# gsgen3d/gsgen

Hardware: AMD Instinct MI355X
Metric: fwd+bwd renders/sec (800x800, 100k Gaussians) (higher is better)
Workload: dtype f32

## Files before the change

### gsgen_amd/csrc/binning.hip

```cpp
#include "common.hpp"
#include "../../include/gsgen_hip.h"
#include <cstdlib>
#include <vector>

#if defined(GSGEN_EMU_KNOBS)
extern "C" unsigned long long gsgen_emu_emit_staged_keys;
unsigned long long gsgen_emu_emit_staged_keys = 0;
#endif

namespace gs {

constexpr int kGroup = 8;
constexpr int kChunk = 2048;

struct GroupGeom {
  int gx0, gy0, tx, ty, tile;
  bool in_grid;
};
__device__ __forceinline__ GroupGeom group_geom(int ntw, int nth) {
  const int ngw = (ntw + kGroup - 1) / kGroup;
  const int g = (int)blockIdx.x;
  GroupGeom q;
  q.gx0 = (g % ngw) * kGroup;
  q.gy0 = (g / ngw) * kGroup;
  const int lane = lane_id();
  q.tx = q.gx0 + (lane & 7);
  q.ty = q.gy0 + (lane >> 3);
  q.in_grid = (q.tx < ntw) && (q.ty < nth);
  q.tile = q.ty * ntw + q.tx;
  return q;
}

constexpr int kPullWaves = 4;
constexpr int kIter = kChunk / (64 * kPullWaves);

__device__ __forceinline__ int rd_lane(int v, int l) { return __builtin_amdgcn_readlane(v, l); }

struct RectRegs {
  int x0[kIter], y0[kIter], x1[kIter], y1[kIter];
};

template <bool EMIT>
__device__ __forceinline__ void
bin_pull_body(uint32_t N, const int *__restrict__ tl, const int *__restrict__ br,
           const float *__restrict__ depth, int ntw, int nth, uint32_t T,
           uint32_t *__restrict__ cnt, uint32_t *__restrict__ wcnt, const uint32_t *__restrict__ tile_off,
           const uint32_t *__restrict__ ctrl, unsigned long long *__restrict__ keys) {
  __shared__ uint32_t s_cnt[kPullWaves][64];
  if (EMIT && ctrl[1] != 0u) return;
  const GroupGeom q = group_geom(ntw, nth);
  const uint32_t chunk = blockIdx.y;
  const int lane = lane_id();
  const int wave = (int)(threadIdx.x >> 6);
  const uint32_t begin = chunk * (uint32_t)kChunk + (uint32_t)wave * (uint32_t)(64 * kIter);
  const uint32_t stop = min(N, chunk * (uint32_t)kChunk + (uint32_t)kChunk);

  RectRegs R;
  unsigned dbits[EMIT ? kIter : 1];
  unsigned long long touch[kIter];
#pragma unroll
  for (int it = 0; it < kIter; ++it) {
    const uint32_t i = begin + (uint32_t)(it * 64 + lane);
    int x0 = 0, y0 = 0, x1 = -1, y1 = -1;
    if (i < stop) {
      const int2 a = *reinterpret_cast<const int2 *>(tl + 2 * (size_t)i);
      const int2 c = *reinterpret_cast<const int2 *>(br + 2 * (size_t)i);
      x0 = max(a.x, 0); y0 = max(a.y, 0); x1 = min(c.x, ntw - 1); y1 = min(c.y, nth - 1);
      if (EMIT) dbits[it] = __float_as_uint(depth[i]);
    } else if (EMIT) {
      dbits[it] = 0u;
    }
    const bool touches = (x1 >= x0) && (y1 >= y0) && (x1 >= q.gx0) && (x0 <= q.gx0 + kGroup - 1) &&
                         (y1 >= q.gy0) && (y0 <= q.gy0 + kGroup - 1);
    touch[it] = __ballot(touches);
    R.x0[it] = x0; R.y0[it] = y0; R.x1[it] = x1; R.y1[it] = y1;
  }
  if (!EMIT) {
    uint32_t running = 0;
#pragma unroll
    for (int it = 0; it < kIter; ++it) {
      unsigned long long m = touch[it];
      while (m != 0ull) {
        const int src = __ffsll((long long)m) - 1;
        m &= (m - 1ull);
        const int rx0 = rd_lane(R.x0[it], src), rx1 = rd_lane(R.x1[it], src);
        const int ry0 = rd_lane(R.y0[it], src), ry1 = rd_lane(R.y1[it], src);
        const bool hit = (q.tx >= rx0) && (q.tx <= rx1) && (q.ty >= ry0) && (q.ty <= ry1);
        running += hit ? 1u : 0u;
      }
    }
    if (q.in_grid) wcnt[((size_t)chunk * kPullWaves + (size_t)wave) * T + q.tile] = running;
    s_cnt[wave][lane] = running;
    __syncthreads();
    if (wave == 0 && q.in_grid)
      cnt[(size_t)chunk * T + q.tile] = s_cnt[0][lane] + s_cnt[1][lane] + s_cnt[2][lane] + s_cnt[3][lane];
    return;
  }
  uint32_t pos = 0;
  if (q.in_grid) {
    pos = tile_off[q.tile] + cnt[(size_t)chunk * T + q.tile];
    for (int w = 0; w < wave; ++w) pos += wcnt[((size_t)chunk * kPullWaves + (size_t)w) * T + q.tile];
  }
#pragma unroll
  for (int it = 0; it < kIter; ++it) {
    unsigned long long m = touch[it];
    const uint32_t i0 = begin + (uint32_t)(it * 64);
    while (m != 0ull) {
      const int src = __ffsll((long long)m) - 1;
      m &= (m - 1ull);
      const int rx0 = rd_lane(R.x0[it], src), rx1 = rd_lane(R.x1[it], src);
      const int ry0 = rd_lane(R.y0[it], src), ry1 = rd_lane(R.y1[it], src);
      const bool hit = (q.tx >= rx0) && (q.tx <= rx1) && (q.ty >= ry0) && (q.ty <= ry1);
      const unsigned db = (unsigned)rd_lane((int)dbits[EMIT ? it : 0], src);
      if (hit) {
        keys[pos] = ((unsigned long long)db << 32) | (unsigned long long)(i0 + (uint32_t)src);
        ++pos;
      }
    }
  }
}

constexpr uint32_t kScanChunkTiles = 64;
template <uint32_t NW>
__device__ __forceinline__ void
scan_chunks_body(uint32_t T, uint32_t nchunks, uint32_t *__restrict__ cnt, uint32_t *__restrict__ tile_count) {
  __shared__ uint32_t s_part[NW][kScanChunkTiles];
  const uint32_t lane = (uint32_t)lane_id(), w = threadIdx.x >> 6;
  const uint32_t t = blockIdx.x * kScanChunkTiles + lane;
  const uint32_t q = (nchunks + NW - 1u) / NW;
  const uint32_t c0 = min(w * q, nchunks), c1 = min(c0 + q, nchunks);
  uint32_t sum = 0;
  if (t < T)
    for (uint32_t c = c0; c < c1; ++c) sum += cnt[(size_t)c * T + t];
  s_part[w][lane] = sum;
  __syncthreads();
  uint32_t run = 0;
  for (uint32_t k = 0; k < w; ++k) run += s_part[k][lane];
  if (t < T) {
    for (uint32_t c = c0; c < c1; ++c) {
      const uint32_t v = cnt[(size_t)c * T + t];
      cnt[(size_t)c * T + t] = run;
      run += v;
    }
    if (w == NW - 1u) tile_count[t] = run;
  }
}

__device__ __forceinline__ uint32_t sat_add_u32(uint32_t a, uint32_t b) {
  const uint32_t s = a + b;
  return s < a ? 0xffffffffu : s;
}

constexpr uint32_t kScanThreads = 256;
__device__ __forceinline__ void report_pair_count(uint32_t *report, uint32_t total, bool overflow) {
  if (report == nullptr) return;
#if defined(__HIP_DEVICE_COMPILE__)
  __hip_atomic_store(report, total, __ATOMIC_RELAXED, __HIP_MEMORY_SCOPE_SYSTEM);
  if (overflow) __hip_atomic_fetch_max(report + 1, total, __ATOMIC_RELAXED, __HIP_MEMORY_SCOPE_SYSTEM);
#else
  report[0] = total;
  if (overflow && report[1] < total) report[1] = total;
#endif
}
__device__ __forceinline__ void
scan_tiles_body(uint32_t T, const uint32_t *__restrict__ tile_count, uint32_t *__restrict__ tile_off,
             uint32_t *__restrict__ ctrl, uint32_t cap, uint32_t *__restrict__ total_out, uint32_t *report = nullptr) {
  __shared__ uint32_t s_part[kScanThreads];
  const uint32_t t = threadIdx.x;
  const uint32_t per = (T + kScanThreads - 1u) / kScanThreads;
  const uint32_t b = min(t * per, T), e = min(b + per, T);
  uint32_t sum = 0;
  for (uint32_t i = b; i < e; ++i) sum = sat_add_u32(sum, tile_count[i]);
  s_part[t] = sum;
  __syncthreads();
  for (uint32_t d = 1; d < kScanThreads; d <<= 1) {
    const uint32_t v = (t >= d) ? s_part[t - d] : 0u;
    __syncthreads();
    s_part[t] = sat_add_u32(s_part[t], v);
    __syncthreads();
  }
  uint32_t run = (t > 0) ? s_part[t - 1] : 0u;
  for (uint32_t i = b; i < e; ++i) {
    tile_off[i] = run;
    run = sat_add_u32(run, tile_count[i]);
  }
  if (t == kScanThreads - 1u) {
    const uint32_t total = s_part[kScanThreads - 1u];
    tile_off[T] = total;
    ctrl[0] = total;
    ctrl[1] = (total > cap) ? 1u : 0u;
    if (total_out != nullptr) *total_out = total;
    report_pair_count(report, total, total > cap);
  }
}

constexpr uint32_t kWaveSortMax = 512;
__device__ __forceinline__ void
order_tiles_body(uint32_t T, const uint32_t *__restrict__ tile_count, uint32_t *__restrict__ tile_order, uint32_t *__restrict__ n_long) {
  __shared__ uint32_t s_hist[256];
  __shared__ uint32_t s_base[256];
  const uint32_t t = threadIdx.x;
  if (t < 256u) s_hist[t] = 0u;
  __syncthreads();
  for (uint32_t i = t; i < T; i += kScanThreads) atomicAdd(&s_hist[255u - min(tile_count[i] >> 3, 255u)], 1u);
  __syncthreads();
  if (t == 0) {
    uint32_t run = 0;
    for (int b = 0; b < 256; ++b) {
      if (b == 256 - (int)(kWaveSortMax >> 3)) *n_long = run;
      s_base[b] = run;
      run += s_hist[b];
    }
  }
  __syncthreads();
  for (uint32_t i = t; i < T; i += kScanThreads) {
    const uint32_t b = 255u - min(tile_count[i] >> 3, 255u);
    tile_order[atomicAdd(&s_base[b], 1u)] = i;
  }
}

typedef unsigned long long u64;
__device__ __forceinline__ void cmpx(u64 &lo, u64 &hi) {
  const u64 a = lo, b = hi;
  const bool sw = a > b;
  lo = sw ? b : a;
  hi = sw ? a : b;
}
template <int K>
__device__ __forceinline__ void cross_step(u64 (&k)[K], int m, bool flip) {
  const int lane = lane_id();
  int top = m;
  top |= top >> 1; top |= top >> 2; top |= top >> 4;
  top = (top + 1) >> 1;
  const bool upper = (lane & top) != 0;
  auto pick = [&](u64 mine, u64 theirs) {
    const bool take = (theirs < mine) != upper;
    const uint32_t lo = take ? (uint32_t)theirs : (uint32_t)mine, hi = take ? (uint32_t)(theirs >> 32) : (uint32_t)(mine >> 32);
    return ((u64)hi << 32) | lo;
  };
  if (flip) {
    if constexpr (K == 1) {
      k[0] = pick(k[0], __shfl_xor(k[0], m, 64));
    } else {
#pragma unroll
      for (int r = 0; r < K / 2; ++r) {
        const u64 a = k[r], b = k[K - 1 - r];
        const u64 oa = __shfl_xor(b, m, 64), ob = __shfl_xor(a, m, 64);
        k[r] = pick(a, oa);
        k[K - 1 - r] = pick(b, ob);
      }
    }
  } else {
#pragma unroll
    for (int r = 0; r < K; ++r) k[r] = pick(k[r], __shfl_xor(k[r], m, 64));
  }
}
template <int K, int J>
__device__ __forceinline__ void local_step(u64 (&k)[K]) {
#pragma unroll
  for (int r = 0; r < K; ++r) {
    if ((r & J) == 0) cmpx(k[r], k[r | J]);
  }
}
template <int K, int J>
__device__ __forceinline__ void local_tail(u64 (&k)[K]) {
  if constexpr (J >= 1) {
    local_step<K, J>(k);
    local_tail<K, J / 2>(k);
  }
}
template <int K, int SIZE>
__device__ __forceinline__ void local_sizes(u64 (&k)[K]) {
  if constexpr (SIZE <= K) {
#pragma unroll
    for (int r = 0; r < K; ++r) {
      const int l = r ^ (SIZE - 1);
      if (l > r) cmpx(k[r], k[l]);
    }
    local_tail<K, SIZE / 4>(k);
    local_sizes<K, SIZE * 2>(k);
  }
}
template <int K>
__device__ __forceinline__ void sort_regs(u64 (&k)[K]) {
  local_sizes<K, 2>(k);
  for (int size = 2 * K; size <= 64 * K; size <<= 1) {
    cross_step<K>(k, size / K - 1, true);
    for (int j = size >> 2; j >= K; j >>= 1) cross_step<K>(k, j / K, false);
    local_tail<K, K / 2>(k);
  }
}
template <int K>
__device__ __forceinline__ void sort_segment_regs(const u64 *__restrict__ keys, int *__restrict__ ids, uint32_t n) {
  const uint32_t lane = (uint32_t)lane_id();
  u64 k[K];
#pragma unroll
  for (int r = 0; r < K; ++r) {
    const uint32_t e = lane * K + r;
    k[r] = (e < n) ? keys[e] : ~0ull;
  }
  sort_regs<K>(k);
#pragma unroll
  for (int r = 0; r < K; ++r) {
    const uint32_t e = lane * K + r;
    if (e < n) ids[e] = (int)(uint32_t)(k[r] & 0xffffffffull);
  }
}
__device__ __forceinline__ void long_pass(u64 *__restrict__ k, uint32_t n, uint32_t p2, uint32_t dist, bool flip) {
  const uint32_t lane = (uint32_t)lane_id();
  const uint32_t half = p2 >> 1;
  for (uint32_t cbase = 0; cbase < half; cbase += 256u) {
    u64 a[4], b[4];
    uint32_t ia[4], ib[4];
#pragma unroll
    for (int u = 0; u < 4; ++u) {
      const uint32_t c = cbase + (uint32_t)u * 64u + lane;
      const uint32_t off = c & (dist - 1u);
      ia[u] = ((c - off) << 1) + off;
      ib[u] = flip ? (ia[u] ^ (2u * dist - 1u)) : (ia[u] + dist);
      const bool live = c < half && ib[u] < n;
      if (!live) ib[u] = 0xffffffffu;
      a[u] = live ? k[ia[u]] : 0ull;
      b[u] = live ? k[ib[u]] : ~0ull;
    }
#pragma unroll
    for (int u = 0; u < 4; ++u)
      if (ib[u] != 0xffffffffu && a[u] > b[u]) { k[ia[u]] = b[u]; k[ib[u]] = a[u]; }
  }
  wave_mem_fence();
}
template <int K>
__device__ __forceinline__ void sort_segment_long(u64 *__restrict__ keys, int *__restrict__ ids, uint32_t n) {
  constexpr uint32_t kBlock = 64u * K;
  const uint32_t lane = (uint32_t)lane_id();
  const uint32_t nblk = (n + kBlock - 1u) / kBlock;
  u64 k[K];
  for (uint32_t blk = 0; blk < nblk; ++blk) {
    const uint32_t e0 = blk * kBlock + lane * K;
#pragma unroll
    for (int r = 0; r < K; ++r) k[r] = (e0 + r < n) ? keys[e0 + r] : ~0ull;
    sort_regs<K>(k);
    if (nblk == 1u) {
#pragma unroll
      for (int r = 0; r < K; ++r)
        if (e0 + r < n) ids[e0 + r] = (int)(uint32_t)(k[r] & 0xffffffffull);
      return;
    }
#pragma unroll
    for (int r = 0; r < K; ++r)
      if (e0 + r < n) keys[e0 + r] = k[r];
  }
  wave_mem_fence();
  uint32_t p2 = kBlock;
  while (p2 < n) p2 <<= 1;
  for (uint32_t size = 2u * kBlock; size <= p2; size <<= 1) {
    long_pass(keys, n, p2, size >> 1, true);
    for (uint32_t j = size >> 2; j >= kBlock; j >>= 1) long_pass(keys, n, p2, j, false);
    const bool last = size == p2;
    for (uint32_t blk = 0; blk < nblk; ++blk) {
      const uint32_t e0 = blk * kBlock + lane * K;
#pragma unroll
      for (int r = 0; r < K; ++r) k[r] = (e0 + r < n) ? keys[e0 + r] : ~0ull;
      for (int j = (int)kBlock / 2; j >= K; j >>= 1) cross_step<K>(k, j / K, false);
      local_tail<K, K / 2>(k);
#pragma unroll
      for (int r = 0; r < K; ++r) {
        if (e0 + r < n) {
          if (last) ids[e0 + r] = (int)(uint32_t)(k[r] & 0xffffffffull);
          else keys[e0 + r] = k[r];
        }
      }
    }
    wave_mem_fence();
  }
}

constexpr int kCoopWaves = 4;
constexpr uint32_t kCoopMax = 2048;
__device__ __forceinline__ void lds_pass(u64 *k, uint32_t p2, uint32_t dist, bool flip) {
  for (uint32_t c = threadIdx.x; c < (p2 >> 1); c += 64u * kCoopWaves) {
    const uint32_t off = c & (dist - 1u);
    const uint32_t i = ((c - off) << 1) + off;
    const uint32_t l = flip ? (i ^ (2u * dist - 1u)) : (i + dist);
    const u64 a = k[i], b = k[l];
    if (a > b) { k[i] = b; k[l] = a; }
  }
  __syncthreads();
}
template <int KW>
__device__ __forceinline__ void sort_segment_coop(const u64 *__restrict__ keys, int *__restrict__ ids, uint32_t n, u64 *s_keys) {
  constexpr uint32_t kBlk = 64u * KW;
  const uint32_t wave = threadIdx.x >> 6, lane = (uint32_t)lane_id();
  const uint32_t e0 = wave * kBlk + lane * KW;
  u64 k[KW];
#pragma unroll
  for (int r = 0; r < KW; ++r) k[r] = (e0 + r < n) ? keys[e0 + r] : ~0ull;
  sort_regs<KW>(k);
  auto to_lds = [&]() {
#pragma unroll
    for (int r = 0; r < KW; ++r) s_keys[e0 + r] = k[r];
    __syncthreads();
  };
  auto tail_in_registers = [&]() {
#pragma unroll
    for (int r = 0; r < KW; ++r) k[r] = s_keys[e0 + r];
    for (int j = (int)kBlk / 2; j >= KW; j >>= 1) cross_step<KW>(k, j / KW, false);
    local_tail<KW, KW / 2>(k);
  };
  to_lds();
  lds_pass(s_keys, 4u * kBlk, kBlk, true);
  tail_in_registers();
  __syncthreads();
  to_lds();
  lds_pass(s_keys, 4u * kBlk, 2u * kBlk, true);
  lds_pass(s_keys, 4u * kBlk, kBlk, false);
  tail_in_registers();
#pragma unroll
  for (int r = 0; r < KW; ++r)
    if (e0 + r < n) ids[e0 + r] = (int)(uint32_t)(k[r] & 0xffffffffull);
}
__device__ __forceinline__ void
sort_tiles_coop_body(uint32_t tile, const uint32_t *__restrict__ tile_off, const uint32_t *__restrict__ ctrl,
                     unsigned long long *__restrict__ keys, int *__restrict__ ids, int *__restrict__ start,
                     int *__restrict__ end, u64 *s_keys) {
  const uint32_t tid = threadIdx.x;
  if (ctrl[1] != 0u) {
    if (tid == 0) { start[tile] = kListOverflow; end[tile] = kListOverflow; }
    return;
  }
  const uint32_t b = tile_off[tile], e = tile_off[tile + 1];
  const uint32_t n = e - b;
  if (tid == 0) {
    start[tile] = n ? (int)b : -1;
    end[tile] = n ? (int)e : -1;
  }
  if (n == 0) return;
  if (n <= 256u || n > kCoopMax) {
    if (tid >= 64u) return;
    if (n <= 64u) sort_segment_regs<1>(keys + b, ids + b, n);
    else if (n <= 128u) sort_segment_regs<2>(keys + b, ids + b, n);
    else if (n <= 256u) sort_segment_regs<4>(keys + b, ids + b, n);
    else sort_segment_long<8>(keys + b, ids + b, n);
    return;
  }
  if (n <= 512u) sort_segment_coop<2>(keys + b, ids + b, n, s_keys);
  else if (n <= 1024u) sort_segment_coop<4>(keys + b, ids + b, n, s_keys);
  else sort_segment_coop<8>(keys + b, ids + b, n, s_keys);
}
__device__ __forceinline__ void
sort_tiles_packed_body(uint32_t slot, uint32_t T, const uint32_t *__restrict__ tile_order, const uint32_t *__restrict__ tile_off,
                       const uint32_t *__restrict__ ctrl, unsigned long long *__restrict__ keys, int *__restrict__ ids,
                       int *__restrict__ start, int *__restrict__ end, u64 *s_keys) {
  const uint32_t n_long = min(ctrl[2], T);
  if (slot < n_long) {
    sort_tiles_coop_body(tile_order[slot], tile_off, ctrl, keys, ids, start, end, s_keys);
    return;
  }
  const uint32_t at = n_long + (slot - n_long) * (uint32_t)kCoopWaves + (threadIdx.x >> 6);
  if (at >= T) return;
  const uint32_t tile = tile_order[at];
  const bool first = lane_id() == 0;
  if (ctrl[1] != 0u) {
    if (first) { start[tile] = kListOverflow; end[tile] = kListOverflow; }
    return;
  }
  const uint32_t b = tile_off[tile], e = tile_off[tile + 1];
  const uint32_t n = e - b;
  if (first) {
    start[tile] = n ? (int)b : -1;
    end[tile] = n ? (int)e : -1;
  }
  if (n == 0) return;
  if (n <= 64u) sort_segment_regs<1>(keys + b, ids + b, n);
  else if (n <= 128u) sort_segment_regs<2>(keys + b, ids + b, n);
  else if (n <= 256u) sort_segment_regs<4>(keys + b, ids + b, n);
  else sort_segment_regs<8>(keys + b, ids + b, n);
}
static_assert(kWaveSortMax <= 512 && kWaveSortMax % 8 == 0 && kWaveSortMax <= 255 * 8, "sort_tiles_packed_body");
__global__ void __launch_bounds__(64 * kCoopWaves)
k_sort_tiles(uint32_t T, const uint32_t *__restrict__ tile_off, const uint32_t *__restrict__ ctrl,
                  unsigned long long *__restrict__ keys, int *__restrict__ ids, int *__restrict__ start,
                  int *__restrict__ end, const uint32_t *__restrict__ tile_order) {
  __shared__ u64 s_keys[kCoopMax];
  if (tile_order != nullptr) sort_tiles_packed_body(blockIdx.x, T, tile_order, tile_off, ctrl, keys, ids, start, end, s_keys);
  else sort_tiles_coop_body(blockIdx.x, tile_off, ctrl, keys, ids, start, end, s_keys);
}
__global__ void __launch_bounds__(64 * kCoopWaves)
k_sort_tiles_views(uint32_t T, uint32_t B, const GeoView *__restrict__ views) {
  __shared__ u64 s_keys[kCoopMax];
  const uint32_t rank = blockIdx.x / B;
  const GeoView v = views[blockIdx.x - rank * B];
  sort_tiles_packed_body(rank, T, v.tile_order, v.tile_off, v.ctrl, v.keys, v.ids, v.start, v.end, s_keys);
}

template <bool EMIT>
__global__ void __launch_bounds__(64 * kPullWaves)
k_bin_pull(uint32_t N, const int *__restrict__ tl, const int *__restrict__ br,
           const float *__restrict__ depth, int ntw, int nth, uint32_t T,
           uint32_t *__restrict__ cnt, uint32_t *__restrict__ wcnt, const uint32_t *__restrict__ tile_off,
           const uint32_t *__restrict__ ctrl, unsigned long long *__restrict__ keys) {
  bin_pull_body<EMIT>(N, tl, br, depth, ntw, nth, T, cnt, wcnt, tile_off, ctrl, keys);
}
template <bool EMIT>
__global__ void __launch_bounds__(64 * kPullWaves)
k_bin_pull_views(uint32_t N, int ntw, int nth, uint32_t T, const GeoView *__restrict__ views) {
  const GeoView v = views[blockIdx.z];
  bin_pull_body<EMIT>(N, v.tl, v.br, v.depth, ntw, nth, T, v.cnt, v.wcnt, v.tile_off, v.ctrl, v.keys);
}
__global__ void __launch_bounds__(1024)
k_scan_chunks(uint32_t T, uint32_t nchunks, uint32_t *__restrict__ cnt, uint32_t *__restrict__ tile_count) {
  scan_chunks_body<16>(T, nchunks, cnt, tile_count);
}
__global__ void __launch_bounds__(256)
k_scan_chunks_views(uint32_t T, uint32_t nchunks, const GeoView *__restrict__ views) {
  const GeoView v = views[blockIdx.y];
  scan_chunks_body<4>(T, nchunks, v.cnt, v.tile_count);
}
__global__ void __launch_bounds__(kScanThreads)
k_scan_order_tiles(uint32_t T, const uint32_t *__restrict__ tile_count, uint32_t *__restrict__ tile_off,
                   uint32_t *__restrict__ ctrl, uint32_t cap, uint32_t *__restrict__ total_out,
                   uint32_t *__restrict__ tile_order, uint32_t *report) {
  scan_tiles_body(T, tile_count, tile_off, ctrl, cap, total_out, report);
  order_tiles_body(T, tile_count, tile_order, ctrl + 2);
}
__global__ void __launch_bounds__(kScanThreads)
k_scan_order_tiles_views(uint32_t T, const GeoView *__restrict__ views) {
  const GeoView v = views[blockIdx.y];
  scan_tiles_body(T, v.tile_count, v.tile_off, v.ctrl, v.cap, v.total, v.report);
  order_tiles_body(T, v.tile_count, v.tile_order, v.ctrl + 2);
}
constexpr int kPushOwn = 12;
constexpr uint32_t kPushMaxTiles = 8192;
constexpr int kPushThreads = 512;
constexpr uint32_t kPushMinWorkgroups = 128;
constexpr uint32_t kPushMinWorkgroupsBatch = 32;
static uint32_t push_min_workgroups(bool batch) {
#if defined(GSGEN_EMU_KNOBS)
  if (const char *e = getenv("GSGEN_BIN_PUSH_MIN_WORKGROUPS")) return (uint32_t)strtoul(e, nullptr, 10);
#endif
  return batch ? kPushMinWorkgroupsBatch : kPushMinWorkgroups;
}
#if !defined(GSGEN_EMIT_STAGE_WORDS)
#define GSGEN_EMIT_STAGE_WORDS 12288
#endif
constexpr uint32_t kEmitStageWords = GSGEN_EMIT_STAGE_WORDS;
constexpr int kEmitIdBits = 11;
static_assert(kChunk == (1 << kEmitIdBits) && kPushMaxTiles <= (1u << (32 - kEmitIdBits)), "a staged word is (tile << 11) | local id");
static_assert(kPushMaxTiles % kPushThreads == 0 && kPushThreads % 64 == 0, "bin_push_body");
#if defined(__HIP_DEVICE_COMPILE__)
#define GS_PUSH_COUNTERS(name) extern __shared__ uint32_t name[]
#else
#define GS_PUSH_COUNTERS(name) __shared__ uint32_t name[kPushMaxTiles + kEmitAuxWords + kEmitStageWords]
#endif
constexpr uint32_t kEmitLdsWords = 16384;
constexpr uint32_t kEmitAuxWords = 16;
static_assert(kPushThreads / 64 <= 14 && kPushMaxTiles + kEmitAuxWords + 64 <= kEmitLdsWords && kEmitStageWords >= 64, "bin_push_body");
__host__ __device__ __forceinline__ uint32_t emit_stage_cap(uint32_t T) { return min(kEmitStageWords, kEmitLdsWords - kEmitAuxWords - T); }
static size_t push_lds_bytes(uint32_t T, bool emit) { return sizeof(uint32_t) * ((size_t)T + (emit ? kEmitAuxWords + emit_stage_cap(T) : 0u)); }
template <bool EMIT>
__device__ __forceinline__ void
bin_push_body(uint32_t N, const int *__restrict__ tl, const int *__restrict__ br, const float *__restrict__ depth, int ntw, int nth,
              uint32_t T, uint32_t *__restrict__ cnt, const uint32_t *__restrict__ tile_count, const uint32_t *__restrict__ tile_off,
              const uint32_t *__restrict__ ctrl, unsigned long long *__restrict__ keys, uint32_t *s_tile) {
  if (EMIT && ctrl[1] != 0u) return;
  const uint32_t chunk = blockIdx.x;
  const uint32_t chunk_base = chunk * (uint32_t)kChunk;
  uint32_t *const crow = cnt + (size_t)chunk * T;
  uint32_t *const s_wsum = s_tile + T, *const s_meta = s_wsum + 14, *const s_stage = s_wsum + kEmitAuxWords;
  const uint32_t stage_cap = emit_stage_cap(T);
  const int lane = lane_id();
  uint32_t n_staged_tiles = 0, n_staged = 0;
  if constexpr (EMIT) {
    const uint32_t *const nrow = (chunk + 1u < gridDim.x) ? crow + T : tile_count;
    for (uint32_t t = threadIdx.x; t < T; t += (uint32_t)kPushThreads) s_tile[t] = nrow[t] - crow[t];
    if (threadIdx.x < 2u) s_meta[threadIdx.x] = 0u;
    __syncthreads();
    const uint32_t per = (T + (uint32_t)kPushThreads - 1u) / (uint32_t)kPushThreads;
    const uint32_t b = min(threadIdx.x * per, T), e = min(b + per, T);
    uint32_t sum = 0;
    for (uint32_t i = b; i < e; ++i) sum += s_tile[i];
    uint32_t inc = sum;
    for (int d = 1; d < 64; d <<= 1) {
      const uint32_t v = __shfl(inc, max(lane - d, 0), 64);
      if (lane >= d) inc += v;
    }
    const uint32_t wave = threadIdx.x >> 6;
    if (lane == 63) s_wsum[wave] = inc;
    __syncthreads();
    uint32_t run = inc - sum;
    for (uint32_t w = 0; w < wave; ++w) run += s_wsum[w];
    uint32_t last_tile = 0, last_end = 0;
    for (uint32_t i = b; i < e; ++i) {
      const uint32_t c = s_tile[i];
      if (run + c <= stage_cap) {
        s_tile[i] = run;
        last_tile = i + 1u; last_end = run + c;
      } else {
        s_tile[i] = tile_off[i] + crow[i];
      }
      run += c;
    }
    if (last_tile != 0u) { atomicMax(&s_meta[0], last_tile); atomicMax(&s_meta[1], last_end); }
    __syncthreads();
    n_staged_tiles = s_meta[0]; n_staged = s_meta[1];
  } else {
    for (uint32_t t = threadIdx.x; t < T; t += (uint32_t)kPushThreads) s_tile[t] = 0u;
    __syncthreads();
  }
  const uint32_t stop = min(N, chunk_base + (uint32_t)kChunk);
  auto visit = [&](int tile, uint32_t id, unsigned dbits) {
    const uint32_t pos = atomicAdd(&s_tile[tile], 1u);
    if (EMIT) {
      if ((uint32_t)tile < n_staged_tiles) {
        if (pos < stage_cap) s_stage[pos] = ((uint32_t)tile << kEmitIdBits) | (id - chunk_base);
      } else {
        keys[pos] = ((unsigned long long)dbits << 32) | (unsigned long long)id;
      }
    }
  };
  for (uint32_t i0 = chunk_base; i0 < stop; i0 += (uint32_t)kPushThreads) {
    const uint32_t i = i0 + threadIdx.x;
    int x0 = 0, y0 = 0, x1 = -1, y1 = -1;
    unsigned db = 0u;
    if (i < stop) {
      const int2 a = *reinterpret_cast<const int2 *>(tl + 2 * (size_t)i);
      const int2 c = *reinterpret_cast<const int2 *>(br + 2 * (size_t)i);
      x0 = max(a.x, 0); y0 = max(a.y, 0); x1 = min(c.x, ntw - 1); y1 = min(c.y, nth - 1);
      if (EMIT) db = __float_as_uint(depth[i]);
    }
    const int rw = x1 - x0 + 1, rh = y1 - y0 + 1;
    const int n = (rw > 0 && rh > 0) ? rw * rh : 0;
    {
      int tx = x0, ty = y0;
      const int own = min(n, kPushOwn);
      for (int k = 0; k < own; ++k) {
        visit(ty * ntw + tx, i, db);
        if (++tx > x1) { tx = x0; ++ty; }
      }
    }
    unsigned long long big = __ballot(n > kPushOwn);
    while (big != 0ull) {
      const int src = __ffsll((long long)big) - 1;
      big &= (big - 1ull);
      const int bx0 = rd_lane(x0, src), by0 = rd_lane(y0, src), bw = rd_lane(rw, src), bn = rd_lane(n, src);
      const uint32_t bid = (uint32_t)rd_lane((int)i, src);
      const unsigned bdb = (unsigned)rd_lane((int)db, src);
      for (int k = kPushOwn + lane; k < bn; k += 64) {
        const int ry = k / bw;
        visit((by0 + ry) * ntw + bx0 + (k - ry * bw), bid, bdb);
      }
    }
  }
  __syncthreads();
  if constexpr (!EMIT) {
    for (uint32_t t = threadIdx.x; t < T; t += (uint32_t)kPushThreads) crow[t] = s_tile[t];
  } else {
    constexpr int kPer = (int)kPushMaxTiles / kPushThreads;
    uint32_t prev[kPer];
#pragma unroll
    for (int k = 0; k < kPer; ++k) {
      const uint32_t t = threadIdx.x + (uint32_t)(k * kPushThreads);
      prev[k] = (t > 0u && t < n_staged_tiles) ? s_tile[t - 1u] : 0u;
    }
    __syncthreads();
#pragma unroll
    for (int k = 0; k < kPer; ++k) {
      const uint32_t t = threadIdx.x + (uint32_t)(k * kPushThreads);
      if (t < n_staged_tiles) s_tile[t] = tile_off[t] + crow[t] - prev[k];
    }
    __syncthreads();
#if defined(GSGEN_EMU_KNOBS)
    if (threadIdx.x == 0) gsgen_emu_emit_staged_keys += n_staged;
#endif
    for (uint32_t j = threadIdx.x; j < n_staged; j += (uint32_t)kPushThreads) {
      const uint32_t w = s_stage[j];
      const uint32_t id = chunk_base + (w & ((1u << kEmitIdBits) - 1u));
      keys[j + s_tile[w >> kEmitIdBits]] = ((unsigned long long)__float_as_uint(depth[id]) << 32) | (unsigned long long)id;
    }
  }
}

template <bool EMIT>
__global__ void __launch_bounds__(kPushThreads)
k_bin_push(uint32_t N, const int *__restrict__ tl, const int *__restrict__ br, const float *__restrict__ depth, int ntw, int nth,
           uint32_t T, uint32_t *__restrict__ cnt, const uint32_t *__restrict__ tile_count, const uint32_t *__restrict__ tile_off,
           const uint32_t *__restrict__ ctrl, unsigned long long *__restrict__ keys) {
  GS_PUSH_COUNTERS(s_tile);
  bin_push_body<EMIT>(N, tl, br, depth, ntw, nth, T, cnt, tile_count, tile_off, ctrl, keys, s_tile);
}
template <bool EMIT>
__global__ void __launch_bounds__(kPushThreads)
k_bin_push_views(uint32_t N, int ntw, int nth, uint32_t T, const GeoView *__restrict__ views) {
  GS_PUSH_COUNTERS(s_tile);
  const GeoView v = views[blockIdx.y];
  bin_push_body<EMIT>(N, v.tl, v.br, v.depth, ntw, nth, T, v.cnt, v.tile_count, v.tile_off, v.ctrl, v.keys, s_tile);
}

template <int P>
__global__ void __launch_bounds__(64) k_selftest_reduce_scatter(const float *__restrict__ in, float *__restrict__ out) {
  float v[P];
  const int lane = lane_id();
#pragma unroll
  for (int i = 0; i < P; ++i) v[i] = in[lane * P + i];
  wave_reduce_scatter<P>(v);
  out[lane] = v[0];
  out[64 + lane] = (float)(scatter_owner<P>(lane) ? scatter_comp<P>(lane) : -1);
}

__global__ void __launch_bounds__(64) k_selftest_reduce_scatter_sep16(const float *__restrict__ in, const float *__restrict__ u,
                                                                      float *__restrict__ out) {
  v2f c[8];
  const int lane = lane_id();
#pragma unroll
  for (int k = 0; k < 8; ++k) c[k] = v2f{in[lane * 16 + 2 * k], in[lane * 16 + 2 * k + 1]};
  out[lane] = wave_reduce_scatter_sep16(c, u[lane]);
  out[64 + lane] = (float)(sep16_owner(lane) ? sep16_comp(lane) : -1);
  out[128 + lane] = (float)sep16_comp(lane);
}

static inline size_t align_up(size_t v, size_t a) { return (v + a - 1) / a * a; }

struct BinWs {
  uint32_t *tile_count, *tile_off, *ctrl, *cnt, *wcnt, *tile_order;
  unsigned long long *keys;
  int *tl, *br;
  uint32_t nchunks;
  size_t bytes;
};
static BinWs carve(void *base, uint32_t N, uint32_t D, uint32_t T, bool with_rects) {
  BinWs w{};
  size_t off = 0;
  char *p = (char *)base;
  auto take = [&](size_t bytes) { void *r = p ? p + off : nullptr; off += align_up(bytes, 256); return r; };
  w.nchunks = (N + kChunk - 1) / kChunk;
  if (w.nchunks == 0) w.nchunks = 1;
  w.tile_count = (uint32_t *)take(sizeof(uint32_t) * ((size_t)T + 4));
  w.ctrl = w.tile_count ? w.tile_count + T : nullptr;
  w.tile_off = (uint32_t *)take(sizeof(uint32_t) * ((size_t)T + 1));
  w.tile_order = (uint32_t *)take(sizeof(uint32_t) * (size_t)(T ? T : 1));
  w.cnt = (uint32_t *)take(sizeof(uint32_t) * (size_t)w.nchunks * T);
  w.wcnt = (uint32_t *)take(sizeof(uint32_t) * (size_t)w.nchunks * kPullWaves * T);
  w.keys = (unsigned long long *)take(sizeof(unsigned long long) * (size_t)(D ? D : 1));
  if (with_rects) {
    w.tl = (int *)take(sizeof(int) * 2 * (size_t)(N ? N : 1));
    w.br = (int *)take(sizeof(int) * 2 * (size_t)(N ? N : 1));
  }
  w.bytes = off;
  return w;
}

static int bin_and_sort(uint32_t N, uint32_t cap, uint32_t nth, uint32_t ntw, const int *tl,
                        const int *br, const float *depth, int *ids, int *start, int *end,
                        const BinWs &w, uint32_t *total_out, hipStream_t s, uint32_t *report = nullptr) {
  const uint32_t T = nth * ntw;
  if (cap > 0x7fffffffu) return GSGEN_EINVAL;
  const uint32_t ngroups = ((ntw + kGroup - 1) / kGroup) * ((nth + kGroup - 1) / kGroup);
  const dim3 gpull(ngroups, w.nchunks);
  const dim3 bpull(64 * kPullWaves);
  const bool push = T <= kPushMaxTiles && w.nchunks >= push_min_workgroups(false);
  if (N == 0) {
    if (hipError_t e = hipMemsetAsync(w.cnt, 0, sizeof(uint32_t) * (size_t)w.nchunks * T, s)) return (int)e;
  } else if (push) {
    hipLaunchKernelGGL((k_bin_push<false>), dim3(w.nchunks), dim3(kPushThreads), push_lds_bytes(T, false), s, N, tl, br, depth, (int)ntw, (int)nth, T, w.cnt,
                       (const uint32_t *)nullptr, (const uint32_t *)nullptr, (const uint32_t *)nullptr, (unsigned long long *)nullptr);
  } else {
    hipLaunchKernelGGL((k_bin_pull<false>), gpull, bpull, 0, s, N, tl, br, depth, (int)ntw, (int)nth, T,
                       w.cnt, w.wcnt, (const uint32_t *)nullptr, (const uint32_t *)nullptr,
                       (unsigned long long *)nullptr);
  }
  hipLaunchKernelGGL(k_scan_chunks, dim3((T + kScanChunkTiles - 1) / kScanChunkTiles), dim3(1024), 0, s, T, w.nchunks,
                     w.cnt, w.tile_count);
  hipLaunchKernelGGL(k_scan_order_tiles, dim3(1), dim3(kScanThreads), 0, s, T, w.tile_count, w.tile_off, w.ctrl, cap, total_out,
                     w.tile_order, report);
  if (N && push)
    hipLaunchKernelGGL((k_bin_push<true>), dim3(w.nchunks), dim3(kPushThreads), push_lds_bytes(T, true), s, N, tl, br, depth, (int)ntw, (int)nth, T, w.cnt,
                       (const uint32_t *)w.tile_count, (const uint32_t *)w.tile_off, (const uint32_t *)w.ctrl, w.keys);
  else if (N)
    hipLaunchKernelGGL((k_bin_pull<true>), gpull, bpull, 0, s, N, tl, br, depth, (int)ntw, (int)nth, T,
                       w.cnt, w.wcnt, w.tile_off, w.ctrl, w.keys);
  hipLaunchKernelGGL(k_sort_tiles, dim3(T), dim3(64 * kCoopWaves), 0, s, T, w.tile_off, w.ctrl, w.keys, ids, start, end,
                     (const uint32_t *)w.tile_order);
  return (int)hipGetLastError();
}

}

using namespace gs;

extern "C" {

int gsgen_internal_frame_project(uint32_t N, const float *mean, const float *qvec, const float *svec,
                                 const float *cam, int w, int h, int ntw, float *mean2d, float *cov2d,
                                 float *depth, uint8_t *mask, int *tl, int *br, gsgen_stream_t stream);

int gsgen_internal_frame_project_views(uint32_t N, const float *mean, const float *qvec, const float *svec,
                                       int w, int h, int ntw, const GeoView *host_views, GeoView *dev_views,
                                       uint32_t B, float *zero_shared, size_t zero_shared_floats, gsgen_stream_t stream);

int gsgen_internal_sort_segments(uint32_t T, const uint32_t *tile_off, const uint32_t *ctrl,
                                 unsigned long long *keys, int *ids, int *start, int *end, gsgen_stream_t stream) {
  hipStream_t s = (hipStream_t)stream;
  if (T == 0) return 0;
  hipLaunchKernelGGL(k_sort_tiles, dim3(T), dim3(64 * kCoopWaves), 0, s, T, tile_off, ctrl, keys, ids, start, end,
                     (const uint32_t *)nullptr);
  return (int)hipGetLastError();
}

const char *gsgen_version(void) { return "gsgen_hip 0.1 (gfx950)"; }

uint32_t gsgen_emit_stage_capacity(void) { return kEmitStageWords; }

int gsgen_selftest_reduce_scatter(uint32_t P, const float *in , float *out ,
                                  gsgen_stream_t stream) {
  hipStream_t s = (hipStream_t)stream;
  switch (P) {
    case 8: hipLaunchKernelGGL((k_selftest_reduce_scatter<8>), dim3(1), dim3(64), 0, s, in, out); break;
    case 16: hipLaunchKernelGGL((k_selftest_reduce_scatter<16>), dim3(1), dim3(64), 0, s, in, out); break;
    case 32: hipLaunchKernelGGL((k_selftest_reduce_scatter<32>), dim3(1), dim3(64), 0, s, in, out); break;
    case 64: hipLaunchKernelGGL((k_selftest_reduce_scatter<64>), dim3(1), dim3(64), 0, s, in, out); break;
    default: return GSGEN_EUNSUPPORTED;
  }
  return (int)hipGetLastError();
}

int gsgen_selftest_reduce_scatter_sep16(const float *in , const float *u , float *out ,
                                        gsgen_stream_t stream) {
  if (in == nullptr || u == nullptr || out == nullptr) return GSGEN_EINVAL;
  hipLaunchKernelGGL(k_selftest_reduce_scatter_sep16, dim3(1), dim3(64), 0, (hipStream_t)stream, in, u, out);
  return (int)hipGetLastError();
}

const char *gsgen_error_string(int code) {
  if (code == 0) return "success";
  if (code == GSGEN_EUNSUPPORTED) return "unsupported configuration (tile_size 1 .. 32 -- 16 only for the batched / segmented / fused entry points --, C in 1..4, kNN K in 1..32)";
  if (code == GSGEN_EINVAL) return "invalid argument (null pointer or inconsistent sizes)";
  if (code == GSGEN_EWORKSPACE) return "workspace too small";
  if (code > 0) return hipGetErrorString((hipError_t)code);
  return "unknown error";
}

size_t gsgen_tile_culling_workspace_bytes(uint32_t N, uint32_t D, uint32_t n_tiles) {
  return carve(nullptr, N, D, n_tiles, false).bytes;
}

int gsgen_tile_culling_aabb_start_end(uint32_t N, uint32_t D, uint32_t n_tiles_h,
                                      uint32_t n_tiles_w, const int *aabb_topleft,
                                      const int *aabb_bottomright, const float *depth,
                                      int *gaussian_ids, int *start, int *end, void *workspace,
                                      size_t workspace_bytes, gsgen_stream_t stream) {
  const uint32_t T = n_tiles_h * n_tiles_w;
  if (T == 0) return 0;
  if (!start || !end || !workspace) return GSGEN_EINVAL;
  if (N && (!aabb_topleft || !aabb_bottomright || !depth)) return GSGEN_EINVAL;
  if (D && !gaussian_ids) return GSGEN_EINVAL;
  if (D > 0x7fffffffu) return GSGEN_EINVAL;
  const BinWs w = carve(workspace, N, D, T, false);
  if (w.bytes > workspace_bytes) return GSGEN_EWORKSPACE;
  return bin_and_sort(N, D, n_tiles_h, n_tiles_w, aabb_topleft, aabb_bottomright, depth, gaussian_ids,
                      start, end, w, nullptr, (hipStream_t)stream);
}

size_t gsgen_frame_batch_workspace_bytes(uint32_t n_views) { return (size_t)n_views * sizeof(GeoView); }

int gsgen_frame_geometry_batch(uint32_t n_views, const gsgen_geometry_view *views, uint32_t N, const float *mean,
                               const float *qvec, const float *svec, uint32_t W, uint32_t H,
                               void *batch_workspace, gsgen_stream_t stream) {
  return gsgen_frame_geometry_batch_zero(n_views, views, N, mean, qvec, svec, W, H, nullptr, 0, batch_workspace, stream);
}

int gsgen_frame_geometry_batch_zero(uint32_t n_views, const gsgen_geometry_view *views, uint32_t N, const float *mean,
                                    const float *qvec, const float *svec, uint32_t W, uint32_t H, float *zero_shared,
                                    size_t zero_shared_floats, void *batch_workspace, gsgen_stream_t stream) {
  if (zero_shared_floats && (!zero_shared || (zero_shared_floats & 3u) || (reinterpret_cast<uintptr_t>(zero_shared) & 15u) ||
                             zero_shared_floats / 4 > 0xffffffffull))
    return GSGEN_EINVAL;
  const uint32_t ntw = (W + kTile - 1) / kTile, nth = (H + kTile - 1) / kTile;
  const uint32_t T = ntw * nth;
  if (T == 0 || n_views == 0) return 0;
  if (!views || !batch_workspace) return GSGEN_EINVAL;
  if (n_views > 65535) return GSGEN_EINVAL;
  if (N && (!mean || !qvec || !svec)) return GSGEN_EINVAL;
  std::vector<GeoView> gv(n_views);
  uint32_t nchunks = 1;
  for (uint32_t b = 0; b < n_views; ++b) {
    const gsgen_geometry_view &v = views[b];
    if (!v.cam || !v.start || !v.end || !v.workspace || !v.total || !v.gaussian_ids) return GSGEN_EINVAL;
    if (N && (!v.mean2d || !v.cov2d || !v.depth || !v.mask)) return GSGEN_EINVAL;
    if (v.D_cap > 0x7fffffffu) return GSGEN_EINVAL;
    const BinWs w = carve(v.workspace, N, v.D_cap, T, true);
    if (w.bytes > v.workspace_bytes) return GSGEN_EWORKSPACE;
    nchunks = w.nchunks;
    GeoView &g = gv[b];
    g.cam = v.cam; g.mean2d = v.mean2d; g.cov2d = v.cov2d; g.depth = v.depth; g.mask = v.mask;
    g.tl = w.tl; g.br = w.br; g.cnt = w.cnt; g.wcnt = w.wcnt; g.tile_count = w.tile_count; g.tile_off = w.tile_off;
    g.ctrl = w.ctrl; g.tile_order = w.tile_order; g.keys = w.keys;
    g.ids = v.gaussian_ids; g.start = v.start; g.end = v.end; g.total = v.total; g.cap = v.D_cap; g.report = v.pair_report;
    g.z_mean2d = v.zero_grad_mean2d; g.z_cov2d = v.zero_grad_cov2d; g.z_chan6 = v.zero_grad_chan6;
    g.chol = v.chol; g.max_r = v.max_radii2d;
    if ((reinterpret_cast<uintptr_t>(g.z_mean2d) & 7u) || (reinterpret_cast<uintptr_t>(g.z_cov2d) & 15u) ||
        (reinterpret_cast<uintptr_t>(g.z_chan6) & 7u) || (reinterpret_cast<uintptr_t>(g.chol) & 15u))
      return GSGEN_EINVAL;
  }
  hipStream_t s = (hipStream_t)stream;
  GeoView *dv = reinterpret_cast<GeoView *>(batch_workspace);
  if (int e = gsgen_internal_frame_project_views(N, mean, qvec, svec, (int)W, (int)H, (int)ntw, gv.data(), dv,
                                                 n_views, zero_shared_floats ? zero_shared : nullptr, zero_shared_floats,
                                                 stream))
    return e;
  const uint32_t B = n_views;
  const uint32_t ngroups = ((ntw + kGroup - 1) / kGroup) * ((nth + kGroup - 1) / kGroup);
  const dim3 gpull(ngroups, nchunks, B), bpull(64 * kPullWaves);
  const bool push = T <= kPushMaxTiles && nchunks * B >= push_min_workgroups(true);
  const dim3 gpush(nchunks, B), bpush(kPushThreads);
  if (N == 0) {
    for (uint32_t b = 0; b < B; ++b)
      if (hipError_t e = hipMemsetAsync(gv[b].cnt, 0, sizeof(uint32_t) * (size_t)nchunks * T, s)) return (int)e;
  } else if (push) {
    hipLaunchKernelGGL((k_bin_push_views<false>), gpush, bpush, push_lds_bytes(T, false), s, N, (int)ntw, (int)nth, T, (const GeoView *)dv);
  } else {
    hipLaunchKernelGGL((k_bin_pull_views<false>), gpull, bpull, 0, s, N, (int)ntw, (int)nth, T, (const GeoView *)dv);
  }
  hipLaunchKernelGGL(k_scan_chunks_views, dim3((T + kScanChunkTiles - 1) / kScanChunkTiles, B), dim3(256), 0, s, T, nchunks, (const GeoView *)dv);
  hipLaunchKernelGGL(k_scan_order_tiles_views, dim3(1, B), dim3(kScanThreads), 0, s, T, (const GeoView *)dv);
  if (N && push)
    hipLaunchKernelGGL((k_bin_push_views<true>), gpush, bpush, push_lds_bytes(T, true), s, N, (int)ntw, (int)nth, T, (const GeoView *)dv);
  else if (N)
    hipLaunchKernelGGL((k_bin_pull_views<true>), gpull, bpull, 0, s, N, (int)ntw, (int)nth, T, (const GeoView *)dv);
  hipLaunchKernelGGL(k_sort_tiles_views, dim3(T * B), dim3(64 * kCoopWaves), 0, s, T, B, (const GeoView *)dv);
  return (int)hipGetLastError();
}

void *gsgen_host_device_pointer(void *pinned_host) {
  void *dev = nullptr;
  if (pinned_host == nullptr || hipHostGetDevicePointer(&dev, pinned_host, 0) != hipSuccess) {
    (void)hipGetLastError();
    return nullptr;
  }
  return dev;
}

const uint32_t *gsgen_frame_tile_order(void *workspace, uint32_t N, uint32_t D_cap, uint32_t n_tiles) {
  return carve(workspace, N, D_cap, n_tiles, true).tile_order;
}

size_t gsgen_frame_workspace_bytes(uint32_t N, uint32_t D_cap, uint32_t n_tiles) {
  return carve(nullptr, N, D_cap, n_tiles, true).bytes;
}

int gsgen_frame_geometry(uint32_t N, const float *mean, const float *qvec, const float *svec,
                         const float *cam, uint32_t W, uint32_t H, uint32_t D_cap, float *mean2d,
                         float *cov2d, float *depth, uint8_t *mask, int *gaussian_ids, int *start,
                         int *end, uint32_t *total, void *workspace, size_t workspace_bytes,
                         gsgen_stream_t stream) {
  return gsgen_frame_geometry_report(N, mean, qvec, svec, cam, W, H, D_cap, mean2d, cov2d, depth, mask, gaussian_ids, start, end,
                                     total, nullptr, workspace, workspace_bytes, stream);
}

int gsgen_frame_geometry_report(uint32_t N, const float *mean, const float *qvec, const float *svec,
                                const float *cam, uint32_t W, uint32_t H, uint32_t D_cap, float *mean2d,
                                float *cov2d, float *depth, uint8_t *mask, int *gaussian_ids, int *start,
                                int *end, uint32_t *total, uint32_t *pair_report, void *workspace, size_t workspace_bytes,
                                gsgen_stream_t stream) {
  const uint32_t ntw = (W + kTile - 1) / kTile, nth = (H + kTile - 1) / kTile;
  const uint32_t T = ntw * nth;
  if (T == 0) return 0;
  if (!cam || !start || !end || !workspace || !total) return GSGEN_EINVAL;
  if (N && (!mean || !qvec || !svec || !mean2d || !cov2d || !depth || !mask)) return GSGEN_EINVAL;
  if (D_cap > 0x7fffffffu) return GSGEN_EINVAL;
  const BinWs w = carve(workspace, N, D_cap, T, true);
  if (w.bytes > workspace_bytes) return GSGEN_EWORKSPACE;
  hipStream_t s = (hipStream_t)stream;
  if (int e = gsgen_internal_frame_project(N, mean, qvec, svec, cam, (int)W, (int)H, (int)ntw, mean2d,
                                           cov2d, depth, mask, w.tl, w.br, stream))
    return e;
  return bin_and_sort(N, D_cap, nth, ntw, w.tl, w.br, depth, gaussian_ids, start, end, w, total, s, pair_report);
}

}
```

Baseline: 7538.

## Sort tiles on packed 32-bit depth+index keys with repair and fallback

Per-tile sorts now sort 32-bit keys that pack the high depth bits with the local index, in place of full 64-bit keys. A short odd-even repair pass across lane boundaries on the gathered 64-bit keys follows, then a verification, with a fallback to the full 64-bit sort if order is still wrong. This halves register and shuffle traffic in the bitonic network but adds a gather, the repair and verification passes, and extra barriers. It also allows a 16-per-lane wave sort when the wave sort limit is 1024.

```diff
diff --git a/gsgen_amd/csrc/binning.hip b/gsgen_amd/csrc/binning.hip
--- a/gsgen_amd/csrc/binning.hip
+++ b/gsgen_amd/csrc/binning.hip
@@ -6,6 +6,8 @@
 #if defined(GSGEN_EMU_KNOBS)
 extern "C" unsigned long long gsgen_emu_emit_staged_keys;
 unsigned long long gsgen_emu_emit_staged_keys = 0;
+extern "C" unsigned long long gsgen_emu_sort_packed_tiles, gsgen_emu_sort_repaired_tiles, gsgen_emu_sort_fallback_tiles;
+unsigned long long gsgen_emu_sort_packed_tiles = 0, gsgen_emu_sort_repaired_tiles = 0, gsgen_emu_sort_fallback_tiles = 0;
 #endif
 
 namespace gs {
@@ -226,17 +228,26 @@
   lo = sw ? b : a;
   hi = sw ? a : b;
 }
-template <int K>
-__device__ __forceinline__ void cross_step(u64 (&k)[K], int m, bool flip) {
+__device__ __forceinline__ void cmpx(uint32_t &lo, uint32_t &hi) {
+  const uint32_t a = lo, b = hi;
+  lo = min(a, b);
+  hi = max(a, b);
+}
+template <int K, typename T>
+__device__ __forceinline__ void cross_step(T (&k)[K], int m, bool flip) {
   const int lane = lane_id();
   int top = m;
   top |= top >> 1; top |= top >> 2; top |= top >> 4;
   top = (top + 1) >> 1;
   const bool upper = (lane & top) != 0;
-  auto pick = [&](u64 mine, u64 theirs) {
+  auto pick = [&](T mine, T theirs) -> T {
     const bool take = (theirs < mine) != upper;
-    const uint32_t lo = take ? (uint32_t)theirs : (uint32_t)mine, hi = take ? (uint32_t)(theirs >> 32) : (uint32_t)(mine >> 32);
-    return ((u64)hi << 32) | lo;
+    if constexpr (sizeof(T) == 4) {
+      return take ? theirs : mine;
+    } else {
+      const uint32_t lo = take ? (uint32_t)theirs : (uint32_t)mine, hi = take ? (uint32_t)(theirs >> 32) : (uint32_t)(mine >> 32);
+      return ((u64)hi << 32) | lo;
+    }
   };
   if (flip) {
     if constexpr (K == 1) {
@@ -244,8 +255,8 @@
     } else {
 #pragma unroll
       for (int r = 0; r < K / 2; ++r) {
-        const u64 a = k[r], b = k[K - 1 - r];
-        const u64 oa = __shfl_xor(b, m, 64), ob = __shfl_xor(a, m, 64);
+        const T a = k[r], b = k[K - 1 - r];
+        const T oa = __shfl_xor(b, m, 64), ob = __shfl_xor(a, m, 64);
         k[r] = pick(a, oa);
         k[K - 1 - r] = pick(b, ob);
       }
@@ -255,22 +266,22 @@
     for (int r = 0; r < K; ++r) k[r] = pick(k[r], __shfl_xor(k[r], m, 64));
   }
 }
-template <int K, int J>
-__device__ __forceinline__ void local_step(u64 (&k)[K]) {
+template <int K, int J, typename T>
+__device__ __forceinline__ void local_step(T (&k)[K]) {
 #pragma unroll
   for (int r = 0; r < K; ++r) {
     if ((r & J) == 0) cmpx(k[r], k[r | J]);
   }
 }
-template <int K, int J>
-__device__ __forceinline__ void local_tail(u64 (&k)[K]) {
+template <int K, int J, typename T>
+__device__ __forceinline__ void local_tail(T (&k)[K]) {
   if constexpr (J >= 1) {
     local_step<K, J>(k);
     local_tail<K, J / 2>(k);
   }
 }
-template <int K, int SIZE>
-__device__ __forceinline__ void local_sizes(u64 (&k)[K]) {
+template <int K, int SIZE, typename T>
+__device__ __forceinline__ void local_sizes(T (&k)[K]) {
   if constexpr (SIZE <= K) {
 #pragma unroll
     for (int r = 0; r < K; ++r) {
@@ -281,8 +292,8 @@
     local_sizes<K, SIZE * 2>(k);
   }
 }
-template <int K>
-__device__ __forceinline__ void sort_regs(u64 (&k)[K]) {
+template <int K, typename T>
+__device__ __forceinline__ void sort_regs(T (&k)[K]) {
   local_sizes<K, 2>(k);
   for (int size = 2 * K; size <= 64 * K; size <<= 1) {
     cross_step<K>(k, size / K - 1, true);
@@ -291,7 +302,7 @@
   }
 }
 template <int K>
-__device__ __forceinline__ void sort_segment_regs(const u64 *__restrict__ keys, int *__restrict__ ids, uint32_t n) {
+__device__ __forceinline__ void sort_segment_regs_full(const u64 *__restrict__ keys, int *__restrict__ ids, uint32_t n) {
   const uint32_t lane = (uint32_t)lane_id();
   u64 k[K];
 #pragma unroll
@@ -305,6 +316,108 @@
     const uint32_t e = lane * K + r;
     if (e < n) ids[e] = (int)(uint32_t)(k[r] & 0xffffffffull);
   }
+}
+
+constexpr int kTieRun = 4;
+#if defined(GSGEN_EMU_KNOBS)
+#define GSGEN_EMU_SORT_TALLY(what) (++what)
+#else
+#define GSGEN_EMU_SORT_TALLY(what) ((void)0)
+#endif
+template <int K, bool COOP>
+__device__ __forceinline__ bool repair_and_verify(u64 (&f)[K], uint32_t s0, uint32_t n, u64 *edge, uint32_t slot, uint32_t nslots) {
+  uint32_t buf = 0;
+  u64 prev_last = 0ull, next_first = ~0ull;
+  auto exchange = [&]() {
+    u64 *e = edge + buf * 2u * nslots;
+    e[slot] = f[0];
+    e[nslots + slot] = f[K - 1];
+    if constexpr (COOP) __syncthreads(); else wave_mem_fence();
+    prev_last = slot ? e[nslots + slot - 1u] : 0ull;
+    next_first = (slot + 1u < nslots) ? e[slot + 1u] : ~0ull;
+    buf ^= 1u;
+  };
+#if defined(GSGEN_EMU_KNOBS)
+  u64 before[K];
+  for (int r = 0; r < K; ++r) before[r] = f[r];
+#endif
+#pragma unroll
+  for (int p = 0; p < kTieRun; ++p) {
+    const bool last_pairs = ((s0 + (uint32_t)K - 1u) & 1u) == (uint32_t)(p & 1);
+    const bool first_pairs = ((s0 - 1u) & 1u) == (uint32_t)(p & 1);
+    if (K == 1 || (p & 1)) exchange();
+#pragma unroll
+    for (int r = 0; r + 1 < K; ++r)
+      if (((K & 1) == 0) ? ((r & 1) == (p & 1)) : true) cmpx(f[r], f[r + 1]);
+    if (K == 1 || (p & 1)) {
+      if (K == 1) {
+        const u64 mine = f[0];
+        if (last_pairs) f[0] = mine < next_first ? mine : next_first;
+        if (first_pairs) f[0] = mine > prev_last ? mine : prev_last;
+      } else {
+        const u64 a = f[0], b = f[K - 1];
+        if (first_pairs) f[0] = a > prev_last ? a : prev_last;
+        if (last_pairs) f[K - 1] = b < next_first ? b : next_first;
+      }
+    }
+  }
+  exchange();
+  bool bad = false;
+#pragma unroll
+  for (int r = 0; r < K; ++r) {
+    const u64 succ = (r + 1 < K) ? f[(r + 1 < K) ? r + 1 : r] : next_first;
+    bad = bad || (s0 + (uint32_t)r + 1u < n && !(f[r] < succ));
+  }
+#if defined(GSGEN_EMU_KNOBS)
+  bool moved = false;
+  for (int r = 0; r < K; ++r) moved = moved || before[r] != f[r];
+  if constexpr (COOP) {
+    const bool any_moved = __syncthreads_or((int)moved) != 0;
+    if (slot == 0 && any_moved) ++gsgen_emu_sort_repaired_tiles;
+  } else {
+    const bool any_moved = wave_any(moved);
+    if (slot == 0 && any_moved) ++gsgen_emu_sort_repaired_tiles;
+  }
+#endif
+  const bool wave_bad = wave_any(bad);
+  if constexpr (COOP) {
+    uint32_t *flag = reinterpret_cast<uint32_t *>(edge + 4u * nslots);
+    if ((slot & 63u) == 0u) flag[slot >> 6] = wave_bad ? 1u : 0u;
+    __syncthreads();
+    uint32_t any_bad = 0u;
+    for (uint32_t w = 0; w < (nslots >> 6); ++w) any_bad |= flag[w];
+    return any_bad == 0u;
+  } else {
+    return !wave_bad;
+  }
+}
+__device__ __forceinline__ uint32_t key_depth_bits(const u64 *__restrict__ keys, uint32_t e) {
+  return reinterpret_cast<const uint32_t *>(keys)[2u * e + 1u];
+}
+template <int K>
+__device__ __forceinline__ void sort_segment_regs(const u64 *__restrict__ keys, int *__restrict__ ids, uint32_t n, u64 *edge) {
+  constexpr uint32_t kP = 64u * K;
+  const uint32_t lane = (uint32_t)lane_id();
+  const uint32_t s0 = lane * K;
+  uint32_t k[K];
+#pragma unroll
+  for (int r = 0; r < K; ++r) {
+    const uint32_t e = s0 + r;
+    k[r] = (e < n) ? ((key_depth_bits(keys, e) & ~(kP - 1u)) | e) : 0xffffffffu;
+  }
+  sort_regs<K>(k);
+  u64 f[K];
+#pragma unroll
+  for (int r = 0; r < K; ++r) f[r] = (s0 + r < n) ? keys[k[r] & (kP - 1u)] : ~0ull;
+  if (lane == 0) GSGEN_EMU_SORT_TALLY(gsgen_emu_sort_packed_tiles);
+  if (!repair_and_verify<K, false>(f, s0, n, edge, lane, 64u)) {
+    if (lane == 0) GSGEN_EMU_SORT_TALLY(gsgen_emu_sort_fallback_tiles);
+    sort_segment_regs_full<K>(keys, ids, n);
+    return;
+  }
+#pragma unroll
+  for (int r = 0; r < K; ++r)
+    if (s0 + r < n) ids[s0 + r] = (int)(uint32_t)(f[r] & 0xffffffffull);
 }
 __device__ __forceinline__ void long_pass(u64 *__restrict__ k, uint32_t n, uint32_t p2, uint32_t dist, bool flip) {
   const uint32_t lane = (uint32_t)lane_id();
@@ -377,18 +490,42 @@
 
 constexpr int kCoopWaves = 4;
 constexpr uint32_t kCoopMax = 2048;
-__device__ __forceinline__ void lds_pass(u64 *k, uint32_t p2, uint32_t dist, bool flip) {
+template <typename T>
+__device__ __forceinline__ void lds_pass(T *k, uint32_t p2, uint32_t dist, bool flip) {
   for (uint32_t c = threadIdx.x; c < (p2 >> 1); c += 64u * kCoopWaves) {
     const uint32_t off = c & (dist - 1u);
     const uint32_t i = ((c - off) << 1) + off;
     const uint32_t l = flip ? (i ^ (2u * dist - 1u)) : (i + dist);
-    const u64 a = k[i], b = k[l];
+    const T a = k[i], b = k[l];
     if (a > b) { k[i] = b; k[l] = a; }
   }
   __syncthreads();
 }
+template <int KW, typename T>
+__device__ __forceinline__ void coop_merge_quarters(T (&k)[KW], uint32_t e0, T *s) {
+  constexpr uint32_t kBlk = 64u * KW;
+  auto to_lds = [&]() {
+#pragma unroll
+    for (int r = 0; r < KW; ++r) s[e0 + r] = k[r];
+    __syncthreads();
+  };
+  auto tail_in_registers = [&]() {
+#pragma unroll
+    for (int r = 0; r < KW; ++r) k[r] = s[e0 + r];
+    for (int j = (int)kBlk / 2; j >= KW; j >>= 1) cross_step<KW>(k, j / KW, false);
+    local_tail<KW, KW / 2>(k);
+  };
+  to_lds();
+  lds_pass(s, 4u * kBlk, kBlk, true);
+  tail_in_registers();
+  __syncthreads();
+  to_lds();
+  lds_pass(s, 4u * kBlk, 2u * kBlk, true);
+  lds_pass(s, 4u * kBlk, kBlk, false);
+  tail_in_registers();
+}
 template <int KW>
-__device__ __forceinline__ void sort_segment_coop(const u64 *__restrict__ keys, int *__restrict__ ids, uint32_t n, u64 *s_keys) {
+__device__ __forceinline__ void sort_segment_coop_full(const u64 *__restrict__ keys, int *__restrict__ ids, uint32_t n, u64 *s_keys) {
   constexpr uint32_t kBlk = 64u * KW;
   const uint32_t wave = threadIdx.x >> 6, lane = (uint32_t)lane_id();
   const uint32_t e0 = wave * kBlk + lane * KW;
@@ -396,29 +533,37 @@
 #pragma unroll
   for (int r = 0; r < KW; ++r) k[r] = (e0 + r < n) ? keys[e0 + r] : ~0ull;
   sort_regs<KW>(k);
-  auto to_lds = [&]() {
-#pragma unroll
-    for (int r = 0; r < KW; ++r) s_keys[e0 + r] = k[r];
-    __syncthreads();
-  };
-  auto tail_in_registers = [&]() {
-#pragma unroll
-    for (int r = 0; r < KW; ++r) k[r] = s_keys[e0 + r];
-    for (int j = (int)kBlk / 2; j >= KW; j >>= 1) cross_step<KW>(k, j / KW, false);
-    local_tail<KW, KW / 2>(k);
-  };
-  to_lds();
-  lds_pass(s_keys, 4u * kBlk, kBlk, true);
-  tail_in_registers();
-  __syncthreads();
-  to_lds();
-  lds_pass(s_keys, 4u * kBlk, 2u * kBlk, true);
-  lds_pass(s_keys, 4u * kBlk, kBlk, false);
-  tail_in_registers();
+  coop_merge_quarters<KW>(k, e0, s_keys);
 #pragma unroll
   for (int r = 0; r < KW; ++r)
     if (e0 + r < n) ids[e0 + r] = (int)(uint32_t)(k[r] & 0xffffffffull);
 }
+template <int KW>
+__device__ __forceinline__ void sort_segment_coop(const u64 *__restrict__ keys, int *__restrict__ ids, uint32_t n, u64 *s_keys) {
+  constexpr uint32_t kBlk = 64u * KW, kP = 4u * kBlk;
+  const uint32_t wave = threadIdx.x >> 6, lane = (uint32_t)lane_id();
+  const uint32_t e0 = wave * kBlk + lane * KW;
+  uint32_t k[KW];
+#pragma unroll
+  for (int r = 0; r < KW; ++r) k[r] = (e0 + r < n) ? ((key_depth_bits(keys, e0 + r) & ~(kP - 1u)) | (e0 + r)) : 0xffffffffu;
+  sort_regs<KW>(k);
+  coop_merge_quarters<KW>(k, e0, reinterpret_cast<uint32_t *>(s_keys));
+  u64 f[KW];
+#pragma unroll
+  for (int r = 0; r < KW; ++r) f[r] = (e0 + r < n) ? keys[k[r] & (kP - 1u)] : ~0ull;
+  if (threadIdx.x == 0) GSGEN_EMU_SORT_TALLY(gsgen_emu_sort_packed_tiles);
+  __syncthreads();
+  if (!repair_and_verify<KW, true>(f, e0, n, s_keys, threadIdx.x, 64u * kCoopWaves)) {
+    if (threadIdx.x == 0) GSGEN_EMU_SORT_TALLY(gsgen_emu_sort_fallback_tiles);
+    __syncthreads();
+    sort_segment_coop_full<KW>(keys, ids, n, s_keys);
+    return;
+  }
+#pragma unroll
+  for (int r = 0; r < KW; ++r)
+    if (e0 + r < n) ids[e0 + r] = (int)(uint32_t)(f[r] & 0xffffffffull);
+}
+static_assert(4u * 64u * kCoopWaves + kCoopWaves <= kCoopMax, "the edge words and flags of a four-wavefront list fit s_keys");
 __device__ __forceinline__ void
 sort_tiles_coop_body(uint32_t tile, const uint32_t *__restrict__ tile_off, const uint32_t *__restrict__ ctrl,
                      unsigned long long *__restrict__ keys, int *__restrict__ ids, int *__restrict__ start,
@@ -437,9 +582,9 @@
   if (n == 0) return;
   if (n <= 256u || n > kCoopMax) {
     if (tid >= 64u) return;
-    if (n <= 64u) sort_segment_regs<1>(keys + b, ids + b, n);
-    else if (n <= 128u) sort_segment_regs<2>(keys + b, ids + b, n);
-    else if (n <= 256u) sort_segment_regs<4>(keys + b, ids + b, n);
+    if (n <= 64u) sort_segment_regs<1>(keys + b, ids + b, n, s_keys);
+    else if (n <= 128u) sort_segment_regs<2>(keys + b, ids + b, n, s_keys);
+    else if (n <= 256u) sort_segment_regs<4>(keys + b, ids + b, n, s_keys);
     else sort_segment_long<8>(keys + b, ids + b, n);
     return;
   }
@@ -471,12 +616,14 @@
     end[tile] = n ? (int)e : -1;
   }
   if (n == 0) return;
-  if (n <= 64u) sort_segment_regs<1>(keys + b, ids + b, n);
-  else if (n <= 128u) sort_segment_regs<2>(keys + b, ids + b, n);
-  else if (n <= 256u) sort_segment_regs<4>(keys + b, ids + b, n);
-  else sort_segment_regs<8>(keys + b, ids + b, n);
-}
-static_assert(kWaveSortMax <= 512 && kWaveSortMax % 8 == 0 && kWaveSortMax <= 255 * 8, "sort_tiles_packed_body");
+  u64 *edge = s_keys + (threadIdx.x >> 6) * (kCoopMax / kCoopWaves);
+  if (n <= 64u) sort_segment_regs<1>(keys + b, ids + b, n, edge);
+  else if (n <= 128u) sort_segment_regs<2>(keys + b, ids + b, n, edge);
+  else if (n <= 256u) sort_segment_regs<4>(keys + b, ids + b, n, edge);
+  else if (kWaveSortMax <= 512u || n <= 512u) sort_segment_regs<8>(keys + b, ids + b, n, edge);
+  else sort_segment_regs<16>(keys + b, ids + b, n, edge);
+}
+static_assert((kWaveSortMax == 512 || kWaveSortMax == 1024) && kWaveSortMax % 8 == 0 && kWaveSortMax <= 255 * 8, "sort_tiles_packed_body");
 __global__ void __launch_bounds__(64 * kCoopWaves)
 k_sort_tiles(uint32_t T, const uint32_t *__restrict__ tile_off, const uint32_t *__restrict__ ctrl,
                   unsigned long long *__restrict__ keys, int *__restrict__ ids, int *__restrict__ start,
```

Result: no change. 7540, median of 3 (+0.0%).
